# googlegenomics/spark-examples

Measured on NVIDIA H100. Metric: genotype-cells/sec (N x V) into Gram, higher is better.
Workload: dtype int8

## Files before the change

spark_examples_b200/csrc/gram_sm90.cu:

```cuda
#include <cuda.h>
#include <cuda_runtime.h>

#include <cstring>

#include <algorithm>
#include <map>
#include <mutex>
#include <tuple>
#include <type_traits>
#include <cstdio>
#include <cstdlib>
#include <string>
#include <vector>

#include "ptx_sm90.cuh"
#include "vpca_internal.h"

namespace vpca {

namespace {

constexpr int kThreads = 384;
constexpr int kKBytes = 128;
constexpr int kBoxRows = 128;
// ... 451 lines not shown
                const int rowA = (CG == 2 && cta_rank != 0) ? s.rowA1 : s.rowA0;
                const bool two_boxes = s.n_eff > kBoxRows;
                const bool self_b = (CG == 2) && (s.flags & kTileSelfB) != 0;
                const uint32_t tx = (uint32_t)((two_boxes ? 2 : 1) + (self_b ? 0 : 1)) * C::BOX_BYTES;
                if (a.sync_lead > 0 && leader && s.win != synced_win) {
                    synced_win = s.win;
                    if (s.win >= a.sync_lead) wait_window(a.win_done, s.win - a.sync_lead, a.active_workers);
                }
                for (int kb = s.kb0; kb < s.kb1; ++kb, ++it) {
                    const uint32_t st = it % C::STAGES, ph = (it / C::STAGES) & 1u;
                    mbar_wait(empty_bar(st), ph ^ 1u, a.err, 1);
                    const int pnl = kb / a.kb_per_panel;
                    const int kc = (kb - pnl * a.kb_per_panel) * a.kc_per_kb;
                    ptx::mbar_arrive_expect_tx(full_bar(st), tx);
                    if constexpr (CG == 2) {
                        if (two_boxes || cta_rank == 0)
                            ptx::tma_load_3d_multicast(sB(st) + cta_rank * C::BOX_BYTES, &tmap, full_bar(st), kc,
                                                       s.rowB + (int)cta_rank * kBoxRows, pnl, 0x3);
                    } else {
                        ptx::tma_load_3d(sB(st), &tmap, full_bar(st), kc, s.rowB, pnl);
                        if (two_boxes) ptx::tma_load_3d(sB(st) + C::BOX_BYTES, &tmap, full_bar(st), kc, s.rowB + kBoxRows, pnl);
                    }
                    if (!self_b) ptx::tma_load_3d(sA(st), &tmap, full_bar(st), kc, rowA, pnl);
                }
                if (a.sync_lead > 0 && leader && s.last_in_win)
                    asm volatile("red.release.gpu.global.add.s32 [%0], 1;" ::"l"(a.win_done + s.win) : "memory");
            }
        }
    } else {
        asm volatile("setmaxnreg.inc.sync.aligned.u32 232;");
        const int cw = (warp >> 2) - 1;
        const int wq = warp & 3;
        const uint32_t ctid = threadIdx.x - 128;
        AccT<KIND> acc[2][64];
        Sched sc;
        sc.init(a, worker);
        Seg s;
        uint32_t it = 0;
        while (sc.next(s)) {
            const bool filler = (CG == 2) && cta_rank != 0 && (s.flags & kTileFiller) != 0;
            const bool self_b = (CG == 2) && (s.flags & kTileSelfB) != 0;
            const int mrow0 = cw * 128;
            const bool act0 = mrow0 < s.n_eff, act1 = mrow0 + 64 < s.n_eff;
            if (s.first) {
#pragma unroll
                for (int i = 0; i < 64; ++i) {
                    acc[0][i] = 0;
                    acc[1][i] = 0;
                }
            }
            const uint32_t a_off = (self_b ? cta_rank : 2u) * (uint32_t)(kBoxRows * 128);
            int pending = -1;
            for (int kb = s.kb0; kb < s.kb1; ++kb, ++it) {
                const uint32_t st = it % C::STAGES, ph = (it / C::STAGES) & 1u;
                mbar_wait(full_bar(st), ph, a.err, 3);
                uint32_t opB, opA;
                if constexpr (KIND == 2) {
                    const uint32_t xb = smem_base + C::STAGES * C::STAGE_BYTES + (it & 1u) * C::XBUF_BYTES;
                    ptx::named_sync(1, 256);
                    const int nb = s.n_eff > kBoxRows ? 2 * kBoxRows : kBoxRows;
                    const int rows = nb + (self_b ? 0 : kBoxRows);
                    for (int c = (int)ctid; c < rows * 8; c += 256) {
                        const int r = c >> 3, j = c & 7;
                        const uint32_t src = (r < nb ? sB(st) + (uint32_t)r * 64u : sA(st) + (uint32_t)(r - nb) * 64u) + (uint32_t)j * 8u;
                        const int xr = r < nb ? r : 2 * kBoxRows + (r - nb);
                        uint32_t lo, hi;
                        asm volatile("ld.shared.v2.u32 {%0, %1}, [%2];" : "=r"(lo), "=r"(hi) : "r"(src));
                        const uint32_t o0 = e2m1x4_to_s8x2(lo & 0xFFFFu), o1 = e2m1x4_to_s8x2(lo >> 16);
                        const uint32_t o2 = e2m1x4_to_s8x2(hi & 0xFFFFu), o3 = e2m1x4_to_s8x2(hi >> 16);
                        const uint32_t dst = xb + (uint32_t)xr * 128u + (((uint32_t)j ^ ((uint32_t)xr & 7u)) << 4);
                        asm volatile("st.shared.v4.u32 [%0], {%1, %2, %3, %4};" ::"r"(dst), "r"(o0), "r"(o1), "r"(o2), "r"(o3)
                                     : "memory");
                    }
                    ptx::fence_proxy_async();
                    ptx::named_sync(1, 256);
                    if (threadIdx.x % 128 == 0) release(st);
                    opB = xb;
                } else {
                    opB = sB(st);
                }
                opA = opB + a_off;
                const uint64_t bdesc = make_smem_desc(opA);
                const uint64_t adesc0 = make_smem_desc(opB + (uint32_t)mrow0 * 128u);
                const uint64_t adesc1 = make_smem_desc(opB + (uint32_t)(mrow0 + 64) * 128u);
                ptx::wgmma_fence_acc(acc[0]);
                ptx::wgmma_fence_acc(acc[1]);
                ptx::wgmma_fence();
#pragma unroll
                for (int k = 0; k < kKBytes / 32; ++k) {
                    if constexpr (KIND == 1) {
                        ptx::wgmma_bf16(acc[0], adesc0 + 2 * k, bdesc + 2 * k);
                        ptx::wgmma_bf16(acc[1], adesc1 + 2 * k, bdesc + 2 * k);
                    } else {
                        ptx::wgmma_s8(acc[0], adesc0 + 2 * k, bdesc + 2 * k);
                        ptx::wgmma_s8(acc[1], adesc1 + 2 * k, bdesc + 2 * k);
                    }
                }
                ptx::wgmma_commit();
                ptx::wgmma_wait<1>();
                ptx::wgmma_fence_acc(acc[0]);
                ptx::wgmma_fence_acc(acc[1]);
                if constexpr (KIND != 2) {
                    if (pending >= 0 && threadIdx.x % 128 == 0) release((uint32_t)pending);
                }
                pending = (int)st;
            }
            ptx::wgmma_wait<0>();
            ptx::wgmma_fence_acc(acc[0]);
            ptx::wgmma_fence_acc(acc[1]);
            if constexpr (KIND != 2) {
                if (pending >= 0 && threadIdx.x % 128 == 0) release((uint32_t)pending);
            }
            if (!s.flush || filler) continue;

            const int colA = (CG == 2 && cta_rank != 0) ? s.rowA1 : s.rowA0;
            const int row_end = min(a.row_limit, s.rowB + s.n_eff);
            const bool pair64 = a.red64 != 0 && (a.n & 1) == 0;
#pragma unroll
            for (int j = 0; j < 2; ++j) {
                if (!(j == 0 ? act0 : act1)) continue;
#pragma unroll
                for (int h = 0; h < 2; ++h) {
                    const int row = s.rowB + mrow0 + 64 * j + 16 * wq + (int)(lane >> 2) + 8 * h;
                    if (row >= row_end) continue;
                    int32_t* own = a.S;
                    if (a.num_peers != 0 && a.peer_mode == 1) {
                        int o = 0;
                        while (o + 1 < a.num_peers && row >= a.own_end[o]) ++o;
                        own = a.peer[o];
                    }
#pragma unroll
                    for (int i = 0; i < 16; ++i) {
                        const int col = colA + 8 * i + 2 * (int)(lane & 3);
                        if (col >= a.n) continue;
                        int v0 = acc_to_int<KIND>(acc[j][4 * i + 2 * h]);
                        int v1 = acc_to_int<KIND>(acc[j][4 * i + 2 * h + 1]);
                        if ((s.flags & kTileXpose) != 0 && (row >> 7) < (col >> 7)) {
                            for (int e = 0; e < 2; ++e) {
                                const int v = e ? v1 : v0, c = col + e;
                                if (v == 0 || c >= a.n) continue;
                                const size_t o = (size_t)c * (size_t)a.n + (size_t)row;
                                if (a.num_peers == 0) {
                                    asm volatile("red.global.add.s32 [%0], %1;" ::"l"(a.S + o), "r"(v) : "memory");
                                } else if (a.peer_mode == 1) {
                                    int q = 0;
                                    while (q + 1 < a.num_peers && c >= a.own_end[q]) ++q;
                                    asm volatile("red.relaxed.sys.global.add.s32 [%0], %1;" ::"l"(a.peer[q] + o), "r"(v) : "memory");
                                } else {
                                    for (int d = 0; d < a.num_peers; ++d)
                                        asm volatile("red.relaxed.sys.global.add.s32 [%0], %1;" ::"l"(a.peer[d] + o), "r"(v)
                                                     : "memory");
                                }
                            }
                            continue;
                        }
                        if (row < col) v0 = 0;
                        if (row < col + 1 || col + 1 >= a.n) v1 = 0;
                        if ((v0 | v1) == 0) continue;
                        const size_t o = (size_t)row * (size_t)a.n + (size_t)col;
                        if (pair64) {
                            const unsigned long long packed = (unsigned long long)(unsigned)v0 | ((unsigned long long)(unsigned)v1 << 32);
                            if (a.num_peers == 0) {
                                asm volatile("red.global.add.u64 [%0], %1;" ::"l"(a.S + o), "l"(packed) : "memory");
                            } else if (a.peer_mode == 1) {
                                asm volatile("red.relaxed.sys.global.add.u64 [%0], %1;" ::"l"(own + o), "l"(packed) : "memory");
                            } else {
                                for (int d = 0; d < a.num_peers; ++d)
                                    asm volatile("red.relaxed.sys.global.add.u64 [%0], %1;" ::"l"(a.peer[d] + o), "l"(packed)
                                                 : "memory");
                            }
                        } else {
                            for (int e = 0; e < 2; ++e) {
                                const int v = e ? v1 : v0;
                                if (v == 0) continue;
                                if (a.num_peers == 0) {
                                    asm volatile("red.global.add.s32 [%0], %1;" ::"l"(a.S + o + e), "r"(v) : "memory");
                                } else if (a.peer_mode == 1) {
                                    asm volatile("red.relaxed.sys.global.add.s32 [%0], %1;" ::"l"(own + o + e), "r"(v) : "memory");
                                } else {
                                    for (int d = 0; d < a.num_peers; ++d)
                                        asm volatile("red.relaxed.sys.global.add.s32 [%0], %1;" ::"l"(a.peer[d] + o + e), "r"(v)
                                                     : "memory");
                                }
                            }
                        }
                    }
                }
            }
        }
        if (a.prof != nullptr && threadIdx.x == 128) a.prof[(size_t)blockIdx.x * 4 + 2] = globaltimer_ns();
    }

    if constexpr (CG == 2) ptx::cluster_sync();
    else __syncthreads();
    if (a.prof != nullptr && threadIdx.x == 0) a.prof[(size_t)blockIdx.x * 4 + 3] = globaltimer_ns();
}

__global__ void rebalance_kernel(const long long* __restrict__ prof, double* __restrict__ cum, int workers, int cta_group,
                                 double gain, double max_share, long long min_ns, int* __restrict__ gen, const TileDesc* __restrict__ tiles,
                                 int num_tiles, int total_weight, int kbw, int col_limit) {
    __shared__ double sh[1024];
    __shared__ double cand[1025];
    __shared__ long long need[1025];
    __shared__ double red_sum, red_min;
    __shared__ int reject, need_repair;
    const int w = threadIdx.x;
    const bool active = w < workers;
    double t = 0.0, share_old = 0.0;
    if (active) {
        const long long t0 = prof[(size_t)w * cta_group * 4 + 0], t1 = prof[(size_t)w * cta_group * 4 + 2];
        t = (double)(t1 - t0);
        share_old = cum[w + 1] - cum[w];
    }
    sh[w] = active ? t : 1e30;
    if (w == 0) {
        reject = 0;
// ... 865 lines not shown
```

spark_examples_b200/csrc/ptx_sm90.cuh:

```cuda
#pragma once
#include <cstdint>
#include <cuda_runtime.h>

namespace vpca {
namespace ptx {

__device__ __forceinline__ uint32_t smem_u32(const void* p) {
    return static_cast<uint32_t>(__cvta_generic_to_shared(p));
}

__device__ __forceinline__ uint32_t lane_id() {
    uint32_t r;
    asm volatile("mov.u32 %0, %%laneid;" : "=r"(r));
    return r;
}

__device__ __forceinline__ bool elect_one() {
    uint32_t pred = 0;
    asm volatile(
        "{\n\t"
        ".reg .pred P;\n\t"
        "elect.sync _|P, 0xffffffff;\n\t"
        "selp.u32 %0, 1, 0, P;\n\t"
        "}\n"
// ... 33 lines not shown
__device__ __forceinline__ void prefetch_tensormap(const void* desc) {
    asm volatile("prefetch.tensormap [%0];" ::"l"(reinterpret_cast<uint64_t>(desc)) : "memory");
}
__device__ __forceinline__ void tma_load_3d(uint32_t smem_dst, const void* desc, uint32_t bar, int32_t c0, int32_t c1,
                                            int32_t c2) {
    asm volatile(
        "cp.async.bulk.tensor.3d.shared::cluster.global.mbarrier::complete_tx::bytes [%0], [%1, {%3, %4, %5}], [%2];"
        ::"r"(smem_dst), "l"(reinterpret_cast<uint64_t>(desc)), "r"(bar), "r"(c0), "r"(c1), "r"(c2)
        : "memory");
}
__device__ __forceinline__ void tma_load_3d_multicast(uint32_t smem_dst, const void* desc, uint32_t bar, int32_t c0,
                                                      int32_t c1, int32_t c2, uint16_t cta_mask) {
    asm volatile(
        "cp.async.bulk.tensor.3d.shared::cluster.global.mbarrier::complete_tx::bytes.multicast::cluster"
        " [%0], [%1, {%3, %4, %5}], [%2], %6;"
        ::"r"(smem_dst), "l"(reinterpret_cast<uint64_t>(desc)), "r"(bar), "r"(c0), "r"(c1), "r"(c2), "h"(cta_mask)
        : "memory");
}
__device__ __forceinline__ uint32_t mapa(uint32_t saddr, uint32_t rank) {
    uint32_t r;
    asm volatile("mapa.shared::cluster.u32 %0, %1, %2;" : "=r"(r) : "r"(saddr), "r"(rank));
    return r;
}
__device__ __forceinline__ void mbar_arrive_cluster(uint32_t cluster_bar) {
    asm volatile("mbarrier.arrive.shared::cluster.b64 _, [%0];" ::"r"(cluster_bar) : "memory");
}
__device__ __forceinline__ void cluster_sync() {
    asm volatile("barrier.cluster.arrive.release;\n\tbarrier.cluster.wait.acquire;" ::: "memory");
}
__device__ __forceinline__ void wgmma_fence() { asm volatile("wgmma.fence.sync.aligned;" ::: "memory"); }
__device__ __forceinline__ void wgmma_commit() { asm volatile("wgmma.commit_group.sync.aligned;" ::: "memory"); }
template <int N>
__device__ __forceinline__ void wgmma_wait() { asm volatile("wgmma.wait_group.sync.aligned %0;" ::"n"(N) : "memory"); }
__device__ __forceinline__ void wgmma_fence_acc(uint32_t (&d)[64]) {
#pragma unroll
    for (int i = 0; i < 64; ++i) asm volatile("" : "+r"(d[i])::"memory");
}
__device__ __forceinline__ void wgmma_fence_acc(float (&d)[64]) {
#pragma unroll
    for (int i = 0; i < 64; ++i) asm volatile("" : "+f"(d[i])::"memory");
}

__device__ __forceinline__ void wgmma_s8(uint32_t (&d)[64], uint64_t a_desc, uint64_t b_desc) {
    asm volatile(
        "{\n\t.reg .pred p;\n\tsetp.ne.b32 p, 1, 0;\n\t"
        "wgmma.mma_async.sync.aligned.m64n128k32.s32.s8.s8 "
        "{%0, %1, %2, %3, %4, %5, %6, %7, %8, %9, %10, %11, %12, %13, %14, %15, %16, %17, %18, %19, %20, %21, %22, %23, %24, %25, %26, %27, %28, %29, %30, %31, %32, %33, %34, %35, %36, %37, %38, %39, %40, %41, %42, %43, %44, %45, %46, %47, %48, %49, %50, %51, %52, %53, %54, %55, %56, %57, %58, %59, %60, %61, %62, %63}, %64, %65, p;\n\t}\n"
        : "+r"(d[0]), "+r"(d[1]), "+r"(d[2]), "+r"(d[3]), "+r"(d[4]), "+r"(d[5]), "+r"(d[6]), "+r"(d[7]), "+r"(d[8]), "+r"(d[9]), "+r"(d[10]), "+r"(d[11]), "+r"(d[12]), "+r"(d[13]), "+r"(d[14]), "+r"(d[15]), "+r"(d[16]), "+r"(d[17]), "+r"(d[18]), "+r"(d[19]), "+r"(d[20]), "+r"(d[21]), "+r"(d[22]), "+r"(d[23]), "+r"(d[24]), "+r"(d[25]), "+r"(d[26]), "+r"(d[27]), "+r"(d[28]), "+r"(d[29]), "+r"(d[30]), "+r"(d[31]), "+r"(d[32]), "+r"(d[33]), "+r"(d[34]), "+r"(d[35]), "+r"(d[36]), "+r"(d[37]), "+r"(d[38]), "+r"(d[39]), "+r"(d[40]), "+r"(d[41]), "+r"(d[42]), "+r"(d[43]), "+r"(d[44]), "+r"(d[45]), "+r"(d[46]), "+r"(d[47]), "+r"(d[48]), "+r"(d[49]), "+r"(d[50]), "+r"(d[51]), "+r"(d[52]), "+r"(d[53]), "+r"(d[54]), "+r"(d[55]), "+r"(d[56]), "+r"(d[57]), "+r"(d[58]), "+r"(d[59]), "+r"(d[60]), "+r"(d[61]), "+r"(d[62]), "+r"(d[63])
        : "l"(a_desc), "l"(b_desc));
}

__device__ __forceinline__ void wgmma_bf16(float (&f)[64], uint64_t a_desc, uint64_t b_desc) {
    asm volatile(
        "{\n\t.reg .pred p;\n\tsetp.ne.b32 p, 1, 0;\n\t"
        "wgmma.mma_async.sync.aligned.m64n128k16.f32.bf16.bf16 "
        "{%0, %1, %2, %3, %4, %5, %6, %7, %8, %9, %10, %11, %12, %13, %14, %15, %16, %17, %18, %19, %20, %21, %22, %23, %24, %25, %26, %27, %28, %29, %30, %31, %32, %33, %34, %35, %36, %37, %38, %39, %40, %41, %42, %43, %44, %45, %46, %47, %48, %49, %50, %51, %52, %53, %54, %55, %56, %57, %58, %59, %60, %61, %62, %63}, %64, %65, p, 1, 1, 0, 0;\n\t}\n"
        : "+f"(f[0]), "+f"(f[1]), "+f"(f[2]), "+f"(f[3]), "+f"(f[4]), "+f"(f[5]), "+f"(f[6]), "+f"(f[7]), "+f"(f[8]), "+f"(f[9]), "+f"(f[10]), "+f"(f[11]), "+f"(f[12]), "+f"(f[13]), "+f"(f[14]), "+f"(f[15]), "+f"(f[16]), "+f"(f[17]), "+f"(f[18]), "+f"(f[19]), "+f"(f[20]), "+f"(f[21]), "+f"(f[22]), "+f"(f[23]), "+f"(f[24]), "+f"(f[25]), "+f"(f[26]), "+f"(f[27]), "+f"(f[28]), "+f"(f[29]), "+f"(f[30]), "+f"(f[31]), "+f"(f[32]), "+f"(f[33]), "+f"(f[34]), "+f"(f[35]), "+f"(f[36]), "+f"(f[37]), "+f"(f[38]), "+f"(f[39]), "+f"(f[40]), "+f"(f[41]), "+f"(f[42]), "+f"(f[43]), "+f"(f[44]), "+f"(f[45]), "+f"(f[46]), "+f"(f[47]), "+f"(f[48]), "+f"(f[49]), "+f"(f[50]), "+f"(f[51]), "+f"(f[52]), "+f"(f[53]), "+f"(f[54]), "+f"(f[55]), "+f"(f[56]), "+f"(f[57]), "+f"(f[58]), "+f"(f[59]), "+f"(f[60]), "+f"(f[61]), "+f"(f[62]), "+f"(f[63])
        : "l"(a_desc), "l"(b_desc));
}

__device__ __forceinline__ void named_sync(uint32_t id, uint32_t count) {
    asm volatile("bar.sync %0, %1;" ::"r"(id), "r"(count) : "memory");
}

}
}
```

Before: 627.6 billion.

## Swap wgmma operand roles to use m64n256 instructions per consumer warpgroup

Each consumer warpgroup now issues one m64n256 wgmma per k-step, with the A-side (64 rows per warpgroup) as the M operand and the full 256-row B block as N. Before, it issued two m64n128 wgmmas sharing a B descriptor. Because the accumulator is now transposed, the epilogue uses a lane-pair shuffle to rebuild adjacent column pairs so the atomic reductions stay paired. The intent is to halve wgmma issue count and make better use of shared-memory operand bandwidth. In exchange the epilogue gets extra shuffles and per-row bounds checks, and tiles with fewer than 256 active rows still compute all 256 columns.

```diff
diff --git a/spark_examples_b200/csrc/gram_sm90.cu b/spark_examples_b200/csrc/gram_sm90.cu
--- a/spark_examples_b200/csrc/gram_sm90.cu
+++ b/spark_examples_b200/csrc/gram_sm90.cu
@@ -507,29 +507,19 @@
         const int cw = (warp >> 2) - 1;
         const int wq = warp & 3;
         const uint32_t ctid = threadIdx.x - 128;
-        AccT<KIND> acc[2][64];
+        AccT<KIND> acc[128];
         Sched sc;
         sc.init(a, worker);
-        Seg s;
+        Seg s{};
         uint32_t it = 0;
-        while (sc.next(s)) {
-            const bool filler = (CG == 2) && cta_rank != 0 && (s.flags & kTileFiller) != 0;
-            const bool self_b = (CG == 2) && (s.flags & kTileSelfB) != 0;
-            const int mrow0 = cw * 128;
-            const bool act0 = mrow0 < s.n_eff, act1 = mrow0 + 64 < s.n_eff;
-            if (s.first) {
-#pragma unroll
-                for (int i = 0; i < 64; ++i) {
-                    acc[0][i] = 0;
-                    acc[1][i] = 0;
-                }
-            }
-            const uint32_t a_off = (self_b ? cta_rank : 2u) * (uint32_t)(kBoxRows * 128);
+        auto consume = [&](auto n_const, uint32_t it, uint32_t a_off, uint32_t b_off, bool self_b) {
+            constexpr int N = decltype(n_const)::value;
             int pending = -1;
-            for (int kb = s.kb0; kb < s.kb1; ++kb, ++it) {
+            const uint32_t it_end = it + (uint32_t)(s.kb1 - s.kb0);
+            for (; it != it_end; ++it) {
                 const uint32_t st = it % C::STAGES, ph = (it / C::STAGES) & 1u;
                 mbar_wait(full_bar(st), ph, a.err, 3);
-                uint32_t opB, opA;
+                uint32_t opB;
                 if constexpr (KIND == 2) {
                     const uint32_t xb = smem_base + C::STAGES * C::STAGE_BYTES + (it & 1u) * C::XBUF_BYTES;
                     ptx::named_sync(1, 256);
@@ -554,109 +544,112 @@
                 } else {
                     opB = sB(st);
                 }
-                opA = opB + a_off;
-                const uint64_t bdesc = make_smem_desc(opA);
-                const uint64_t adesc0 = make_smem_desc(opB + (uint32_t)mrow0 * 128u);
-                const uint64_t adesc1 = make_smem_desc(opB + (uint32_t)(mrow0 + 64) * 128u);
-                ptx::wgmma_fence_acc(acc[0]);
-                ptx::wgmma_fence_acc(acc[1]);
-                ptx::wgmma_fence();
+                if constexpr (N > 0) {
+                    const uint64_t adesc = make_smem_desc(opB + a_off);
+                    const uint64_t bdesc = make_smem_desc(opB + b_off);
+                    ptx::wgmma_fence_acc<N>(acc);
+                    ptx::wgmma_fence();
 #pragma unroll
-                for (int k = 0; k < kKBytes / 32; ++k) {
-                    if constexpr (KIND == 1) {
-                        ptx::wgmma_bf16(acc[0], adesc0 + 2 * k, bdesc + 2 * k);
-                        ptx::wgmma_bf16(acc[1], adesc1 + 2 * k, bdesc + 2 * k);
-                    } else {
-                        ptx::wgmma_s8(acc[0], adesc0 + 2 * k, bdesc + 2 * k);
-                        ptx::wgmma_s8(acc[1], adesc1 + 2 * k, bdesc + 2 * k);
+                    for (int k = 0; k < kKBytes / 32; ++k) {
+                        if constexpr (KIND == 1) ptx::wgmma_bf16<N>(acc, adesc + 2 * k, bdesc + 2 * k);
+                        else ptx::wgmma_s8<N>(acc, adesc + 2 * k, bdesc + 2 * k);
                     }
+                    ptx::wgmma_commit();
+                    ptx::wgmma_wait<1>();
+                    ptx::wgmma_fence_acc<N>(acc);
                 }
-                ptx::wgmma_commit();
-                ptx::wgmma_wait<1>();
-                ptx::wgmma_fence_acc(acc[0]);
-                ptx::wgmma_fence_acc(acc[1]);
                 if constexpr (KIND != 2) {
                     if (pending >= 0 && threadIdx.x % 128 == 0) release((uint32_t)pending);
                 }
                 pending = (int)st;
             }
-            ptx::wgmma_wait<0>();
-            ptx::wgmma_fence_acc(acc[0]);
-            ptx::wgmma_fence_acc(acc[1]);
+            if constexpr (N > 0) {
+                ptx::wgmma_wait<0>();
+                ptx::wgmma_fence_acc<N>(acc);
+            }
             if constexpr (KIND != 2) {
                 if (pending >= 0 && threadIdx.x % 128 == 0) release((uint32_t)pending);
             }
+            return it;
+        };
+        while (sc.next(s)) {
+            const bool filler = (CG == 2) && cta_rank != 0 && (s.flags & kTileFiller) != 0;
+            const bool self_b = (CG == 2) && (s.flags & kTileSelfB) != 0;
+            if (s.first) {
+#pragma unroll
+                for (int i = 0; i < 128; ++i) acc[i] = 0;
+            }
+            const uint32_t a_off = ((self_b ? cta_rank : 2u) * (uint32_t)kBoxRows + (uint32_t)(64 * cw)) * 128u;
+            it = consume(std::integral_constant<int, 256>{}, it, a_off, 0u, self_b);
             if (!s.flush || filler) continue;
 
-            const int colA = (CG == 2 && cta_rank != 0) ? s.rowA1 : s.rowA0;
+            const int colA = ((CG == 2 && cta_rank != 0) ? s.rowA1 : s.rowA0) + 64 * cw;
             const int row_end = min(a.row_limit, s.rowB + s.n_eff);
             const bool pair64 = a.red64 != 0 && (a.n & 1) == 0;
+            const uint32_t odd = (lane >> 2) & 1u;
 #pragma unroll
-            for (int j = 0; j < 2; ++j) {
-                if (!(j == 0 ? act0 : act1)) continue;
+            for (int i = 0; i < 32; ++i) {
+                if (s.rowB + 8 * i >= row_end) break;
 #pragma unroll
                 for (int h = 0; h < 2; ++h) {
-                    const int row = s.rowB + mrow0 + 64 * j + 16 * wq + (int)(lane >> 2) + 8 * h;
-                    if (row >= row_end) continue;
+                    const int m0 = acc_to_int<KIND>(acc[4 * i + 2 * h]), m1 = acc_to_int<KIND>(acc[4 * i + 2 * h + 1]);
+                    const int got = __shfl_xor_sync(0xffffffffu, odd ? m0 : m1, 4);
+                    int v0 = odd ? got : m0, v1 = odd ? m1 : got;
+                    const int row = s.rowB + 8 * i + 2 * (int)(lane & 3) + (int)odd;
+                    const int col = colA + 16 * wq + (int)((lane >> 2) & ~1u) + 8 * h;
+                    if (row >= row_end || col >= a.n) continue;
                     int32_t* own = a.S;
                     if (a.num_peers != 0 && a.peer_mode == 1) {
                         int o = 0;
                         while (o + 1 < a.num_peers && row >= a.own_end[o]) ++o;
                         own = a.peer[o];
                     }
-#pragma unroll
-                    for (int i = 0; i < 16; ++i) {
-                        const int col = colA + 8 * i + 2 * (int)(lane & 3);
-                        if (col >= a.n) continue;
-                        int v0 = acc_to_int<KIND>(acc[j][4 * i + 2 * h]);
-                        int v1 = acc_to_int<KIND>(acc[j][4 * i + 2 * h + 1]);
-                        if ((s.flags & kTileXpose) != 0 && (row >> 7) < (col >> 7)) {
-                            for (int e = 0; e < 2; ++e) {
-                                const int v = e ? v1 : v0, c = col + e;
-                                if (v == 0 || c >= a.n) continue;
-                                const size_t o = (size_t)c * (size_t)a.n + (size_t)row;
-                                if (a.num_peers == 0) {
-                                    asm volatile("red.global.add.s32 [%0], %1;" ::"l"(a.S + o), "r"(v) : "memory");
-                                } else if (a.peer_mode == 1) {
-                                    int q = 0;
-                                    while (q + 1 < a.num_peers && c >= a.own_end[q]) ++q;
-                                    asm volatile("red.relaxed.sys.global.add.s32 [%0], %1;" ::"l"(a.peer[q] + o), "r"(v) : "memory");
-                                } else {
-                                    for (int d = 0; d < a.num_peers; ++d)
-                                        asm volatile("red.relaxed.sys.global.add.s32 [%0], %1;" ::"l"(a.peer[d] + o), "r"(v)
-                                                     : "memory");
-                                }
-                            }
-                            continue;
-                        }
-                        if (row < col) v0 = 0;
-                        if (row < col + 1 || col + 1 >= a.n) v1 = 0;
-                        if ((v0 | v1) == 0) continue;
-                        const size_t o = (size_t)row * (size_t)a.n + (size_t)col;
-                        if (pair64) {
-                            const unsigned long long packed = (unsigned long long)(unsigned)v0 | ((unsigned long long)(unsigned)v1 << 32);
+                    if ((s.flags & kTileXpose) != 0 && (row >> 7) < (col >> 7)) {
+                        for (int e = 0; e < 2; ++e) {
+                            const int v = e ? v1 : v0, c = col + e;
+                            if (v == 0 || c >= a.n) continue;
+                            const size_t o = (size_t)c * (size_t)a.n + (size_t)row;
                             if (a.num_peers == 0) {
-                                asm volatile("red.global.add.u64 [%0], %1;" ::"l"(a.S + o), "l"(packed) : "memory");
+                                asm volatile("red.global.add.s32 [%0], %1;" ::"l"(a.S + o), "r"(v) : "memory");
                             } else if (a.peer_mode == 1) {
-                                asm volatile("red.relaxed.sys.global.add.u64 [%0], %1;" ::"l"(own + o), "l"(packed) : "memory");
+                                int q = 0;
+                                while (q + 1 < a.num_peers && c >= a.own_end[q]) ++q;
+                                asm volatile("red.relaxed.sys.global.add.s32 [%0], %1;" ::"l"(a.peer[q] + o), "r"(v) : "memory");
                             } else {
                                 for (int d = 0; d < a.num_peers; ++d)
-                                    asm volatile("red.relaxed.sys.global.add.u64 [%0], %1;" ::"l"(a.peer[d] + o), "l"(packed)
+                                    asm volatile("red.relaxed.sys.global.add.s32 [%0], %1;" ::"l"(a.peer[d] + o), "r"(v)
                                                  : "memory");
                             }
+                        }
+                        continue;
+                    }
+                    if (row < col) v0 = 0;
+                    if (row < col + 1 || col + 1 >= a.n) v1 = 0;
+                    if ((v0 | v1) == 0) continue;
+                    const size_t o = (size_t)row * (size_t)a.n + (size_t)col;
+                    if (pair64) {
+                        const unsigned long long packed = (unsigned long long)(unsigned)v0 | ((unsigned long long)(unsigned)v1 << 32);
+                        if (a.num_peers == 0) {
+                            asm volatile("red.global.add.u64 [%0], %1;" ::"l"(a.S + o), "l"(packed) : "memory");
+                        } else if (a.peer_mode == 1) {
+                            asm volatile("red.relaxed.sys.global.add.u64 [%0], %1;" ::"l"(own + o), "l"(packed) : "memory");
                         } else {
-                            for (int e = 0; e < 2; ++e) {
-                                const int v = e ? v1 : v0;
-                                if (v == 0) continue;
-                                if (a.num_peers == 0) {
-                                    asm volatile("red.global.add.s32 [%0], %1;" ::"l"(a.S + o + e), "r"(v) : "memory");
-                                } else if (a.peer_mode == 1) {
-                                    asm volatile("red.relaxed.sys.global.add.s32 [%0], %1;" ::"l"(own + o + e), "r"(v) : "memory");
-                                } else {
-                                    for (int d = 0; d < a.num_peers; ++d)
-                                        asm volatile("red.relaxed.sys.global.add.s32 [%0], %1;" ::"l"(a.peer[d] + o + e), "r"(v)
-                                                     : "memory");
-                                }
+                            for (int d = 0; d < a.num_peers; ++d)
+                                asm volatile("red.relaxed.sys.global.add.u64 [%0], %1;" ::"l"(a.peer[d] + o), "l"(packed)
+                                             : "memory");
+                        }
+                    } else {
+                        for (int e = 0; e < 2; ++e) {
+                            const int v = e ? v1 : v0;
+                            if (v == 0) continue;
+                            if (a.num_peers == 0) {
+                                asm volatile("red.global.add.s32 [%0], %1;" ::"l"(a.S + o + e), "r"(v) : "memory");
+                            } else if (a.peer_mode == 1) {
+                                asm volatile("red.relaxed.sys.global.add.s32 [%0], %1;" ::"l"(own + o + e), "r"(v) : "memory");
+                            } else {
+                                for (int d = 0; d < a.num_peers; ++d)
+                                    asm volatile("red.relaxed.sys.global.add.s32 [%0], %1;" ::"l"(a.peer[d] + o + e), "r"(v)
+                                                 : "memory");
                             }
                         }
                     }
diff --git a/spark_examples_b200/csrc/ptx_sm90.cuh b/spark_examples_b200/csrc/ptx_sm90.cuh
--- a/spark_examples_b200/csrc/ptx_sm90.cuh
+++ b/spark_examples_b200/csrc/ptx_sm90.cuh
@@ -89,32 +89,72 @@
 __device__ __forceinline__ void wgmma_commit() { asm volatile("wgmma.commit_group.sync.aligned;" ::: "memory"); }
 template <int N>
 __device__ __forceinline__ void wgmma_wait() { asm volatile("wgmma.wait_group.sync.aligned %0;" ::"n"(N) : "memory"); }
-__device__ __forceinline__ void wgmma_fence_acc(uint32_t (&d)[64]) {
+template <int N>
+__device__ __forceinline__ void wgmma_fence_acc(uint32_t (&d)[128]) {
 #pragma unroll
-    for (int i = 0; i < 64; ++i) asm volatile("" : "+r"(d[i])::"memory");
+    for (int i = 0; i < N / 2; ++i) asm volatile("" : "+r"(d[i])::"memory");
 }
-__device__ __forceinline__ void wgmma_fence_acc(float (&d)[64]) {
+template <int N>
+__device__ __forceinline__ void wgmma_fence_acc(float (&d)[128]) {
 #pragma unroll
-    for (int i = 0; i < 64; ++i) asm volatile("" : "+f"(d[i])::"memory");
+    for (int i = 0; i < N / 2; ++i) asm volatile("" : "+f"(d[i])::"memory");
 }
 
-__device__ __forceinline__ void wgmma_s8(uint32_t (&d)[64], uint64_t a_desc, uint64_t b_desc) {
-    asm volatile(
-        "{\n\t.reg .pred p;\n\tsetp.ne.b32 p, 1, 0;\n\t"
-        "wgmma.mma_async.sync.aligned.m64n128k32.s32.s8.s8 "
-        "{%0, %1, %2, %3, %4, %5, %6, %7, %8, %9, %10, %11, %12, %13, %14, %15, %16, %17, %18, %19, %20, %21, %22, %23, %24, %25, %26, %27, %28, %29, %30, %31, %32, %33, %34, %35, %36, %37, %38, %39, %40, %41, %42, %43, %44, %45, %46, %47, %48, %49, %50, %51, %52, %53, %54, %55, %56, %57, %58, %59, %60, %61, %62, %63}, %64, %65, p;\n\t}\n"
-        : "+r"(d[0]), "+r"(d[1]), "+r"(d[2]), "+r"(d[3]), "+r"(d[4]), "+r"(d[5]), "+r"(d[6]), "+r"(d[7]), "+r"(d[8]), "+r"(d[9]), "+r"(d[10]), "+r"(d[11]), "+r"(d[12]), "+r"(d[13]), "+r"(d[14]), "+r"(d[15]), "+r"(d[16]), "+r"(d[17]), "+r"(d[18]), "+r"(d[19]), "+r"(d[20]), "+r"(d[21]), "+r"(d[22]), "+r"(d[23]), "+r"(d[24]), "+r"(d[25]), "+r"(d[26]), "+r"(d[27]), "+r"(d[28]), "+r"(d[29]), "+r"(d[30]), "+r"(d[31]), "+r"(d[32]), "+r"(d[33]), "+r"(d[34]), "+r"(d[35]), "+r"(d[36]), "+r"(d[37]), "+r"(d[38]), "+r"(d[39]), "+r"(d[40]), "+r"(d[41]), "+r"(d[42]), "+r"(d[43]), "+r"(d[44]), "+r"(d[45]), "+r"(d[46]), "+r"(d[47]), "+r"(d[48]), "+r"(d[49]), "+r"(d[50]), "+r"(d[51]), "+r"(d[52]), "+r"(d[53]), "+r"(d[54]), "+r"(d[55]), "+r"(d[56]), "+r"(d[57]), "+r"(d[58]), "+r"(d[59]), "+r"(d[60]), "+r"(d[61]), "+r"(d[62]), "+r"(d[63])
-        : "l"(a_desc), "l"(b_desc));
+#define VPCA_WG_D16 "%0, %1, %2, %3, %4, %5, %6, %7"
+#define VPCA_WG_D32 VPCA_WG_D16 ", %8, %9, %10, %11, %12, %13, %14, %15"
+#define VPCA_WG_D48 VPCA_WG_D32 ", %16, %17, %18, %19, %20, %21, %22, %23"
+#define VPCA_WG_D64 VPCA_WG_D48 ", %24, %25, %26, %27, %28, %29, %30, %31"
+#define VPCA_WG_D80 VPCA_WG_D64 ", %32, %33, %34, %35, %36, %37, %38, %39"
+#define VPCA_WG_D96 VPCA_WG_D80 ", %40, %41, %42, %43, %44, %45, %46, %47"
+#define VPCA_WG_D112 VPCA_WG_D96 ", %48, %49, %50, %51, %52, %53, %54, %55"
+#define VPCA_WG_D128 VPCA_WG_D112 ", %56, %57, %58, %59, %60, %61, %62, %63"
+#define VPCA_WG_D144 VPCA_WG_D128 ", %64, %65, %66, %67, %68, %69, %70, %71"
+#define VPCA_WG_D160 VPCA_WG_D144 ", %72, %73, %74, %75, %76, %77, %78, %79"
+#define VPCA_WG_D176 VPCA_WG_D160 ", %80, %81, %82, %83, %84, %85, %86, %87"
+#define VPCA_WG_D192 VPCA_WG_D176 ", %88, %89, %90, %91, %92, %93, %94, %95"
+#define VPCA_WG_D208 VPCA_WG_D192 ", %96, %97, %98, %99, %100, %101, %102, %103"
+#define VPCA_WG_D224 VPCA_WG_D208 ", %104, %105, %106, %107, %108, %109, %110, %111"
+#define VPCA_WG_D240 VPCA_WG_D224 ", %112, %113, %114, %115, %116, %117, %118, %119"
+#define VPCA_WG_D256 VPCA_WG_D240 ", %120, %121, %122, %123, %124, %125, %126, %127"
+#define VPCA_WG_OP8(C, d, i) C(d[i]), C(d[i + 1]), C(d[i + 2]), C(d[i + 3]), C(d[i + 4]), C(d[i + 5]), C(d[i + 6]), C(d[i + 7])
+#define VPCA_WG_OPS(C, d)                                                                                                  \
+    VPCA_WG_OP8(C, d, 0), VPCA_WG_OP8(C, d, 8), VPCA_WG_OP8(C, d, 16), VPCA_WG_OP8(C, d, 24), VPCA_WG_OP8(C, d, 32),      \
+        VPCA_WG_OP8(C, d, 40), VPCA_WG_OP8(C, d, 48), VPCA_WG_OP8(C, d, 56), VPCA_WG_OP8(C, d, 64), VPCA_WG_OP8(C, d, 72), \
+        VPCA_WG_OP8(C, d, 80), VPCA_WG_OP8(C, d, 88), VPCA_WG_OP8(C, d, 96), VPCA_WG_OP8(C, d, 104),                      \
+        VPCA_WG_OP8(C, d, 112), VPCA_WG_OP8(C, d, 120)
+#define VPCA_WG_S8(NN)                                                                                         \
+    if constexpr (N == NN)                                                                                     \
+        asm volatile("{\n\t.reg .pred p;\n\tsetp.ne.b32 p, 1, 0;\n\t"                                          \
+                     "wgmma.mma_async.sync.aligned.m64n" #NN "k32.s32.s8.s8 {" VPCA_WG_D##NN "}, %128, %129, p;\n\t}\n" \
+                     : VPCA_WG_OPS("+r", d)                                                                    \
+                     : "l"(a_desc), "l"(b_desc));
+#define VPCA_WG_BF16(NN)                                                                                       \
+    if constexpr (N == NN)                                                                                     \
+        asm volatile("{\n\t.reg .pred p;\n\tsetp.ne.b32 p, 1, 0;\n\t"                                          \
+                     "wgmma.mma_async.sync.aligned.m64n" #NN "k16.f32.bf16.bf16 {" VPCA_WG_D##NN                \
+                     "}, %128, %129, p, 1, 1, 0, 0;\n\t}\n"                                                    \
+                     : VPCA_WG_OPS("+f", f)                                                                    \
+                     : "l"(a_desc), "l"(b_desc));
+
+template <int N>
+__device__ __forceinline__ void wgmma_s8(uint32_t (&d)[128], uint64_t a_desc, uint64_t b_desc) {
+    static_assert(N % 16 == 0 && N >= 16 && N <= 256, "wgmma_s8: N is a multiple of 16 in [16, 256]");
+    VPCA_WG_S8(16) VPCA_WG_S8(32) VPCA_WG_S8(48) VPCA_WG_S8(64) VPCA_WG_S8(80) VPCA_WG_S8(96) VPCA_WG_S8(112)
+    VPCA_WG_S8(128) VPCA_WG_S8(144) VPCA_WG_S8(160) VPCA_WG_S8(176) VPCA_WG_S8(192) VPCA_WG_S8(208) VPCA_WG_S8(224)
+    VPCA_WG_S8(240) VPCA_WG_S8(256)
 }
 
-__device__ __forceinline__ void wgmma_bf16(float (&f)[64], uint64_t a_desc, uint64_t b_desc) {
-    asm volatile(
-        "{\n\t.reg .pred p;\n\tsetp.ne.b32 p, 1, 0;\n\t"
-        "wgmma.mma_async.sync.aligned.m64n128k16.f32.bf16.bf16 "
-        "{%0, %1, %2, %3, %4, %5, %6, %7, %8, %9, %10, %11, %12, %13, %14, %15, %16, %17, %18, %19, %20, %21, %22, %23, %24, %25, %26, %27, %28, %29, %30, %31, %32, %33, %34, %35, %36, %37, %38, %39, %40, %41, %42, %43, %44, %45, %46, %47, %48, %49, %50, %51, %52, %53, %54, %55, %56, %57, %58, %59, %60, %61, %62, %63}, %64, %65, p, 1, 1, 0, 0;\n\t}\n"
-        : "+f"(f[0]), "+f"(f[1]), "+f"(f[2]), "+f"(f[3]), "+f"(f[4]), "+f"(f[5]), "+f"(f[6]), "+f"(f[7]), "+f"(f[8]), "+f"(f[9]), "+f"(f[10]), "+f"(f[11]), "+f"(f[12]), "+f"(f[13]), "+f"(f[14]), "+f"(f[15]), "+f"(f[16]), "+f"(f[17]), "+f"(f[18]), "+f"(f[19]), "+f"(f[20]), "+f"(f[21]), "+f"(f[22]), "+f"(f[23]), "+f"(f[24]), "+f"(f[25]), "+f"(f[26]), "+f"(f[27]), "+f"(f[28]), "+f"(f[29]), "+f"(f[30]), "+f"(f[31]), "+f"(f[32]), "+f"(f[33]), "+f"(f[34]), "+f"(f[35]), "+f"(f[36]), "+f"(f[37]), "+f"(f[38]), "+f"(f[39]), "+f"(f[40]), "+f"(f[41]), "+f"(f[42]), "+f"(f[43]), "+f"(f[44]), "+f"(f[45]), "+f"(f[46]), "+f"(f[47]), "+f"(f[48]), "+f"(f[49]), "+f"(f[50]), "+f"(f[51]), "+f"(f[52]), "+f"(f[53]), "+f"(f[54]), "+f"(f[55]), "+f"(f[56]), "+f"(f[57]), "+f"(f[58]), "+f"(f[59]), "+f"(f[60]), "+f"(f[61]), "+f"(f[62]), "+f"(f[63])
-        : "l"(a_desc), "l"(b_desc));
+template <int N>
+__device__ __forceinline__ void wgmma_bf16(float (&f)[128], uint64_t a_desc, uint64_t b_desc) {
+    static_assert(N % 16 == 0 && N >= 16 && N <= 256, "wgmma_bf16: N is a multiple of 16 in [16, 256]");
+    VPCA_WG_BF16(16) VPCA_WG_BF16(32) VPCA_WG_BF16(48) VPCA_WG_BF16(64) VPCA_WG_BF16(80) VPCA_WG_BF16(96)
+    VPCA_WG_BF16(112) VPCA_WG_BF16(128) VPCA_WG_BF16(144) VPCA_WG_BF16(160) VPCA_WG_BF16(176) VPCA_WG_BF16(192)
+    VPCA_WG_BF16(208) VPCA_WG_BF16(224) VPCA_WG_BF16(240) VPCA_WG_BF16(256)
 }
+#undef VPCA_WG_S8
+#undef VPCA_WG_BF16
+#undef VPCA_WG_OPS
+#undef VPCA_WG_OP8
 
 __device__ __forceinline__ void named_sync(uint32_t id, uint32_t count) {
     asm volatile("bar.sync %0, %1;" ::"r"(id), "r"(count) : "memory");
```

After: 642.8 billion (median of 6 runs). 2.4% higher.

## Switch consumer WGMMA to m64n256 with swapped operand roles and transposed epilogue

Applied to the files above, without the earlier changes.

Each consumer warpgroup now issues one m64n256k32 WGMMA per k-step instead of two m64n128 instructions. The roles flip: the 128-row A tile supplies 64 rows per warpgroup and the full 256-row B panel becomes the N dimension. This halves the WGMMA instruction count and cuts redundant shared-memory reads of the shared operand. The accumulator is now transposed relative to the output, so the epilogue uses a lane-xor-4 shuffle to rebuild adjacent column pairs for the packed 64-bit reductions. The cost is more complex epilogue indexing, and per-row masking based on n_eff no longer skips whole inactive 64-row halves.

```diff
diff --git a/spark_examples_b200/csrc/gram_sm90.cu b/spark_examples_b200/csrc/gram_sm90.cu
--- a/spark_examples_b200/csrc/gram_sm90.cu
+++ b/spark_examples_b200/csrc/gram_sm90.cu
@@ -507,7 +507,7 @@
         const int cw = (warp >> 2) - 1;
         const int wq = warp & 3;
         const uint32_t ctid = threadIdx.x - 128;
-        AccT<KIND> acc[2][64];
+        AccT<KIND> acc[128];
         Sched sc;
         sc.init(a, worker);
         Seg s;
@@ -515,14 +515,9 @@
         while (sc.next(s)) {
             const bool filler = (CG == 2) && cta_rank != 0 && (s.flags & kTileFiller) != 0;
             const bool self_b = (CG == 2) && (s.flags & kTileSelfB) != 0;
-            const int mrow0 = cw * 128;
-            const bool act0 = mrow0 < s.n_eff, act1 = mrow0 + 64 < s.n_eff;
             if (s.first) {
 #pragma unroll
-                for (int i = 0; i < 64; ++i) {
-                    acc[0][i] = 0;
-                    acc[1][i] = 0;
-                }
+                for (int i = 0; i < 128; ++i) acc[i] = 0;
             }
             const uint32_t a_off = (self_b ? cta_rank : 2u) * (uint32_t)(kBoxRows * 128);
             int pending = -1;
@@ -555,34 +550,25 @@
                     opB = sB(st);
                 }
                 opA = opB + a_off;
-                const uint64_t bdesc = make_smem_desc(opA);
-                const uint64_t adesc0 = make_smem_desc(opB + (uint32_t)mrow0 * 128u);
-                const uint64_t adesc1 = make_smem_desc(opB + (uint32_t)(mrow0 + 64) * 128u);
-                ptx::wgmma_fence_acc(acc[0]);
-                ptx::wgmma_fence_acc(acc[1]);
+                const uint64_t adesc = make_smem_desc(opA + (uint32_t)cw * 64u * 128u);
+                const uint64_t bdesc = make_smem_desc(opB);
+                ptx::wgmma_fence_acc(acc);
                 ptx::wgmma_fence();
 #pragma unroll
                 for (int k = 0; k < kKBytes / 32; ++k) {
-                    if constexpr (KIND == 1) {
-                        ptx::wgmma_bf16(acc[0], adesc0 + 2 * k, bdesc + 2 * k);
-                        ptx::wgmma_bf16(acc[1], adesc1 + 2 * k, bdesc + 2 * k);
-                    } else {
-                        ptx::wgmma_s8(acc[0], adesc0 + 2 * k, bdesc + 2 * k);
-                        ptx::wgmma_s8(acc[1], adesc1 + 2 * k, bdesc + 2 * k);
-                    }
+                    if constexpr (KIND == 1) ptx::wgmma_bf16(acc, adesc + 2 * k, bdesc + 2 * k);
+                    else ptx::wgmma_s8(acc, adesc + 2 * k, bdesc + 2 * k);
                 }
                 ptx::wgmma_commit();
                 ptx::wgmma_wait<1>();
-                ptx::wgmma_fence_acc(acc[0]);
-                ptx::wgmma_fence_acc(acc[1]);
+                ptx::wgmma_fence_acc(acc);
                 if constexpr (KIND != 2) {
                     if (pending >= 0 && threadIdx.x % 128 == 0) release((uint32_t)pending);
                 }
                 pending = (int)st;
             }
             ptx::wgmma_wait<0>();
-            ptx::wgmma_fence_acc(acc[0]);
-            ptx::wgmma_fence_acc(acc[1]);
+            ptx::wgmma_fence_acc(acc);
             if constexpr (KIND != 2) {
                 if (pending >= 0 && threadIdx.x % 128 == 0) release((uint32_t)pending);
             }
@@ -591,72 +577,71 @@
             const int colA = (CG == 2 && cta_rank != 0) ? s.rowA1 : s.rowA0;
             const int row_end = min(a.row_limit, s.rowB + s.n_eff);
             const bool pair64 = a.red64 != 0 && (a.n & 1) == 0;
+            const bool upper = (lane & 4u) != 0;
 #pragma unroll
-            for (int j = 0; j < 2; ++j) {
-                if (!(j == 0 ? act0 : act1)) continue;
+            for (int h = 0; h < 2; ++h) {
+                const int col = colA + 64 * cw + 16 * wq + (int)((lane >> 2) & ~1u) + 8 * h;
 #pragma unroll
-                for (int h = 0; h < 2; ++h) {
-                    const int row = s.rowB + mrow0 + 64 * j + 16 * wq + (int)(lane >> 2) + 8 * h;
-                    if (row >= row_end) continue;
+                for (int i = 0; i < 64; ++i) {
+                    const int c0 = acc_to_int<KIND>(acc[4 * i + 2 * h]);
+                    const int c1 = acc_to_int<KIND>(acc[4 * i + 2 * h + 1]);
+                    const int peer = __shfl_xor_sync(0xffffffffu, upper ? c0 : c1, 4);
+                    int v0 = upper ? peer : c0;
+                    int v1 = upper ? c1 : peer;
+                    const int row = s.rowB + 8 * i + 2 * (int)(lane & 3) + (upper ? 1 : 0);
+                    if (row >= row_end || col >= a.n) continue;
+                    if ((s.flags & kTileXpose) != 0 && (row >> 7) < (col >> 7)) {
+                        for (int e = 0; e < 2; ++e) {
+                            const int v = e ? v1 : v0, c = col + e;
+                            if (v == 0 || c >= a.n) continue;
+                            const size_t o = (size_t)(unsigned)c * (unsigned)a.n + (unsigned)row;
+                            if (a.num_peers == 0) {
+                                asm volatile("red.global.add.s32 [%0], %1;" ::"l"(a.S + o), "r"(v) : "memory");
+                            } else if (a.peer_mode == 1) {
+                                int q = 0;
+                                while (q + 1 < a.num_peers && c >= a.own_end[q]) ++q;
+                                asm volatile("red.relaxed.sys.global.add.s32 [%0], %1;" ::"l"(a.peer[q] + o), "r"(v) : "memory");
+                            } else {
+                                for (int d = 0; d < a.num_peers; ++d)
+                                    asm volatile("red.relaxed.sys.global.add.s32 [%0], %1;" ::"l"(a.peer[d] + o), "r"(v)
+                                                 : "memory");
+                            }
+                        }
+                        continue;
+                    }
+                    if (row < col) v0 = 0;
+                    if (row < col + 1 || col + 1 >= a.n) v1 = 0;
+                    if ((v0 | v1) == 0) continue;
                     int32_t* own = a.S;
                     if (a.num_peers != 0 && a.peer_mode == 1) {
                         int o = 0;
                         while (o + 1 < a.num_peers && row >= a.own_end[o]) ++o;
                         own = a.peer[o];
                     }
-#pragma unroll
-                    for (int i = 0; i < 16; ++i) {
-                        const int col = colA + 8 * i + 2 * (int)(lane & 3);
-                        if (col >= a.n) continue;
-                        int v0 = acc_to_int<KIND>(acc[j][4 * i + 2 * h]);
-                        int v1 = acc_to_int<KIND>(acc[j][4 * i + 2 * h + 1]);
-                        if ((s.flags & kTileXpose) != 0 && (row >> 7) < (col >> 7)) {
-                            for (int e = 0; e < 2; ++e) {
-                                const int v = e ? v1 : v0, c = col + e;
-                                if (v == 0 || c >= a.n) continue;
-                                const size_t o = (size_t)c * (size_t)a.n + (size_t)row;
-                                if (a.num_peers == 0) {
-                                    asm volatile("red.global.add.s32 [%0], %1;" ::"l"(a.S + o), "r"(v) : "memory");
-                                } else if (a.peer_mode == 1) {
-                                    int q = 0;
-                                    while (q + 1 < a.num_peers && c >= a.own_end[q]) ++q;
-                                    asm volatile("red.relaxed.sys.global.add.s32 [%0], %1;" ::"l"(a.peer[q] + o), "r"(v) : "memory");
-                                } else {
-                                    for (int d = 0; d < a.num_peers; ++d)
-                                        asm volatile("red.relaxed.sys.global.add.s32 [%0], %1;" ::"l"(a.peer[d] + o), "r"(v)
-                                                     : "memory");
-                                }
-                            }
-                            continue;
+                    const size_t o = (size_t)(unsigned)row * (unsigned)a.n + (unsigned)col;
+                    if (pair64) {
+                        const unsigned long long packed = (unsigned long long)(unsigned)v0 | ((unsigned long long)(unsigned)v1 << 32);
+                        if (a.num_peers == 0) {
+                            asm volatile("red.global.add.u64 [%0], %1;" ::"l"(a.S + o), "l"(packed) : "memory");
+                        } else if (a.peer_mode == 1) {
+                            asm volatile("red.relaxed.sys.global.add.u64 [%0], %1;" ::"l"(own + o), "l"(packed) : "memory");
+                        } else {
+                            for (int d = 0; d < a.num_peers; ++d)
+                                asm volatile("red.relaxed.sys.global.add.u64 [%0], %1;" ::"l"(a.peer[d] + o), "l"(packed)
+                                             : "memory");
                         }
-                        if (row < col) v0 = 0;
-                        if (row < col + 1 || col + 1 >= a.n) v1 = 0;
-                        if ((v0 | v1) == 0) continue;
-                        const size_t o = (size_t)row * (size_t)a.n + (size_t)col;
-                        if (pair64) {
-                            const unsigned long long packed = (unsigned long long)(unsigned)v0 | ((unsigned long long)(unsigned)v1 << 32);
+                    } else {
+                        for (int e = 0; e < 2; ++e) {
+                            const int v = e ? v1 : v0;
+                            if (v == 0) continue;
                             if (a.num_peers == 0) {
-                                asm volatile("red.global.add.u64 [%0], %1;" ::"l"(a.S + o), "l"(packed) : "memory");
+                                asm volatile("red.global.add.s32 [%0], %1;" ::"l"(a.S + o + e), "r"(v) : "memory");
                             } else if (a.peer_mode == 1) {
-                                asm volatile("red.relaxed.sys.global.add.u64 [%0], %1;" ::"l"(own + o), "l"(packed) : "memory");
+                                asm volatile("red.relaxed.sys.global.add.s32 [%0], %1;" ::"l"(own + o + e), "r"(v) : "memory");
                             } else {
                                 for (int d = 0; d < a.num_peers; ++d)
-                                    asm volatile("red.relaxed.sys.global.add.u64 [%0], %1;" ::"l"(a.peer[d] + o), "l"(packed)
+                                    asm volatile("red.relaxed.sys.global.add.s32 [%0], %1;" ::"l"(a.peer[d] + o + e), "r"(v)
                                                  : "memory");
-                            }
-                        } else {
-                            for (int e = 0; e < 2; ++e) {
-                                const int v = e ? v1 : v0;
-                                if (v == 0) continue;
-                                if (a.num_peers == 0) {
-                                    asm volatile("red.global.add.s32 [%0], %1;" ::"l"(a.S + o + e), "r"(v) : "memory");
-                                } else if (a.peer_mode == 1) {
-                                    asm volatile("red.relaxed.sys.global.add.s32 [%0], %1;" ::"l"(own + o + e), "r"(v) : "memory");
-                                } else {
-                                    for (int d = 0; d < a.num_peers; ++d)
-                                        asm volatile("red.relaxed.sys.global.add.s32 [%0], %1;" ::"l"(a.peer[d] + o + e), "r"(v)
-                                                     : "memory");
-                                }
                             }
                         }
                     }
diff --git a/spark_examples_b200/csrc/ptx_sm90.cuh b/spark_examples_b200/csrc/ptx_sm90.cuh
--- a/spark_examples_b200/csrc/ptx_sm90.cuh
+++ b/spark_examples_b200/csrc/ptx_sm90.cuh
@@ -89,30 +89,30 @@
 __device__ __forceinline__ void wgmma_commit() { asm volatile("wgmma.commit_group.sync.aligned;" ::: "memory"); }
 template <int N>
 __device__ __forceinline__ void wgmma_wait() { asm volatile("wgmma.wait_group.sync.aligned %0;" ::"n"(N) : "memory"); }
-__device__ __forceinline__ void wgmma_fence_acc(uint32_t (&d)[64]) {
+__device__ __forceinline__ void wgmma_fence_acc(uint32_t (&d)[128]) {
 #pragma unroll
-    for (int i = 0; i < 64; ++i) asm volatile("" : "+r"(d[i])::"memory");
+    for (int i = 0; i < 128; ++i) asm volatile("" : "+r"(d[i])::"memory");
 }
-__device__ __forceinline__ void wgmma_fence_acc(float (&d)[64]) {
+__device__ __forceinline__ void wgmma_fence_acc(float (&d)[128]) {
 #pragma unroll
-    for (int i = 0; i < 64; ++i) asm volatile("" : "+f"(d[i])::"memory");
+    for (int i = 0; i < 128; ++i) asm volatile("" : "+f"(d[i])::"memory");
 }
 
-__device__ __forceinline__ void wgmma_s8(uint32_t (&d)[64], uint64_t a_desc, uint64_t b_desc) {
+__device__ __forceinline__ void wgmma_s8(uint32_t (&d)[128], uint64_t a_desc, uint64_t b_desc) {
     asm volatile(
         "{\n\t.reg .pred p;\n\tsetp.ne.b32 p, 1, 0;\n\t"
-        "wgmma.mma_async.sync.aligned.m64n128k32.s32.s8.s8 "
-        "{%0, %1, %2, %3, %4, %5, %6, %7, %8, %9, %10, %11, %12, %13, %14, %15, %16, %17, %18, %19, %20, %21, %22, %23, %24, %25, %26, %27, %28, %29, %30, %31, %32, %33, %34, %35, %36, %37, %38, %39, %40, %41, %42, %43, %44, %45, %46, %47, %48, %49, %50, %51, %52, %53, %54, %55, %56, %57, %58, %59, %60, %61, %62, %63}, %64, %65, p;\n\t}\n"
-        : "+r"(d[0]), "+r"(d[1]), "+r"(d[2]), "+r"(d[3]), "+r"(d[4]), "+r"(d[5]), "+r"(d[6]), "+r"(d[7]), "+r"(d[8]), "+r"(d[9]), "+r"(d[10]), "+r"(d[11]), "+r"(d[12]), "+r"(d[13]), "+r"(d[14]), "+r"(d[15]), "+r"(d[16]), "+r"(d[17]), "+r"(d[18]), "+r"(d[19]), "+r"(d[20]), "+r"(d[21]), "+r"(d[22]), "+r"(d[23]), "+r"(d[24]), "+r"(d[25]), "+r"(d[26]), "+r"(d[27]), "+r"(d[28]), "+r"(d[29]), "+r"(d[30]), "+r"(d[31]), "+r"(d[32]), "+r"(d[33]), "+r"(d[34]), "+r"(d[35]), "+r"(d[36]), "+r"(d[37]), "+r"(d[38]), "+r"(d[39]), "+r"(d[40]), "+r"(d[41]), "+r"(d[42]), "+r"(d[43]), "+r"(d[44]), "+r"(d[45]), "+r"(d[46]), "+r"(d[47]), "+r"(d[48]), "+r"(d[49]), "+r"(d[50]), "+r"(d[51]), "+r"(d[52]), "+r"(d[53]), "+r"(d[54]), "+r"(d[55]), "+r"(d[56]), "+r"(d[57]), "+r"(d[58]), "+r"(d[59]), "+r"(d[60]), "+r"(d[61]), "+r"(d[62]), "+r"(d[63])
+        "wgmma.mma_async.sync.aligned.m64n256k32.s32.s8.s8 "
+        "{%0, %1, %2, %3, %4, %5, %6, %7, %8, %9, %10, %11, %12, %13, %14, %15, %16, %17, %18, %19, %20, %21, %22, %23, %24, %25, %26, %27, %28, %29, %30, %31, %32, %33, %34, %35, %36, %37, %38, %39, %40, %41, %42, %43, %44, %45, %46, %47, %48, %49, %50, %51, %52, %53, %54, %55, %56, %57, %58, %59, %60, %61, %62, %63, %64, %65, %66, %67, %68, %69, %70, %71, %72, %73, %74, %75, %76, %77, %78, %79, %80, %81, %82, %83, %84, %85, %86, %87, %88, %89, %90, %91, %92, %93, %94, %95, %96, %97, %98, %99, %100, %101, %102, %103, %104, %105, %106, %107, %108, %109, %110, %111, %112, %113, %114, %115, %116, %117, %118, %119, %120, %121, %122, %123, %124, %125, %126, %127}, %128, %129, p;\n\t}\n"
+        : "+r"(d[0]), "+r"(d[1]), "+r"(d[2]), "+r"(d[3]), "+r"(d[4]), "+r"(d[5]), "+r"(d[6]), "+r"(d[7]), "+r"(d[8]), "+r"(d[9]), "+r"(d[10]), "+r"(d[11]), "+r"(d[12]), "+r"(d[13]), "+r"(d[14]), "+r"(d[15]), "+r"(d[16]), "+r"(d[17]), "+r"(d[18]), "+r"(d[19]), "+r"(d[20]), "+r"(d[21]), "+r"(d[22]), "+r"(d[23]), "+r"(d[24]), "+r"(d[25]), "+r"(d[26]), "+r"(d[27]), "+r"(d[28]), "+r"(d[29]), "+r"(d[30]), "+r"(d[31]), "+r"(d[32]), "+r"(d[33]), "+r"(d[34]), "+r"(d[35]), "+r"(d[36]), "+r"(d[37]), "+r"(d[38]), "+r"(d[39]), "+r"(d[40]), "+r"(d[41]), "+r"(d[42]), "+r"(d[43]), "+r"(d[44]), "+r"(d[45]), "+r"(d[46]), "+r"(d[47]), "+r"(d[48]), "+r"(d[49]), "+r"(d[50]), "+r"(d[51]), "+r"(d[52]), "+r"(d[53]), "+r"(d[54]), "+r"(d[55]), "+r"(d[56]), "+r"(d[57]), "+r"(d[58]), "+r"(d[59]), "+r"(d[60]), "+r"(d[61]), "+r"(d[62]), "+r"(d[63]), "+r"(d[64]), "+r"(d[65]), "+r"(d[66]), "+r"(d[67]), "+r"(d[68]), "+r"(d[69]), "+r"(d[70]), "+r"(d[71]), "+r"(d[72]), "+r"(d[73]), "+r"(d[74]), "+r"(d[75]), "+r"(d[76]), "+r"(d[77]), "+r"(d[78]), "+r"(d[79]), "+r"(d[80]), "+r"(d[81]), "+r"(d[82]), "+r"(d[83]), "+r"(d[84]), "+r"(d[85]), "+r"(d[86]), "+r"(d[87]), "+r"(d[88]), "+r"(d[89]), "+r"(d[90]), "+r"(d[91]), "+r"(d[92]), "+r"(d[93]), "+r"(d[94]), "+r"(d[95]), "+r"(d[96]), "+r"(d[97]), "+r"(d[98]), "+r"(d[99]), "+r"(d[100]), "+r"(d[101]), "+r"(d[102]), "+r"(d[103]), "+r"(d[104]), "+r"(d[105]), "+r"(d[106]), "+r"(d[107]), "+r"(d[108]), "+r"(d[109]), "+r"(d[110]), "+r"(d[111]), "+r"(d[112]), "+r"(d[113]), "+r"(d[114]), "+r"(d[115]), "+r"(d[116]), "+r"(d[117]), "+r"(d[118]), "+r"(d[119]), "+r"(d[120]), "+r"(d[121]), "+r"(d[122]), "+r"(d[123]), "+r"(d[124]), "+r"(d[125]), "+r"(d[126]), "+r"(d[127])
         : "l"(a_desc), "l"(b_desc));
 }
 
-__device__ __forceinline__ void wgmma_bf16(float (&f)[64], uint64_t a_desc, uint64_t b_desc) {
+__device__ __forceinline__ void wgmma_bf16(float (&f)[128], uint64_t a_desc, uint64_t b_desc) {
     asm volatile(
         "{\n\t.reg .pred p;\n\tsetp.ne.b32 p, 1, 0;\n\t"
-        "wgmma.mma_async.sync.aligned.m64n128k16.f32.bf16.bf16 "
-        "{%0, %1, %2, %3, %4, %5, %6, %7, %8, %9, %10, %11, %12, %13, %14, %15, %16, %17, %18, %19, %20, %21, %22, %23, %24, %25, %26, %27, %28, %29, %30, %31, %32, %33, %34, %35, %36, %37, %38, %39, %40, %41, %42, %43, %44, %45, %46, %47, %48, %49, %50, %51, %52, %53, %54, %55, %56, %57, %58, %59, %60, %61, %62, %63}, %64, %65, p, 1, 1, 0, 0;\n\t}\n"
-        : "+f"(f[0]), "+f"(f[1]), "+f"(f[2]), "+f"(f[3]), "+f"(f[4]), "+f"(f[5]), "+f"(f[6]), "+f"(f[7]), "+f"(f[8]), "+f"(f[9]), "+f"(f[10]), "+f"(f[11]), "+f"(f[12]), "+f"(f[13]), "+f"(f[14]), "+f"(f[15]), "+f"(f[16]), "+f"(f[17]), "+f"(f[18]), "+f"(f[19]), "+f"(f[20]), "+f"(f[21]), "+f"(f[22]), "+f"(f[23]), "+f"(f[24]), "+f"(f[25]), "+f"(f[26]), "+f"(f[27]), "+f"(f[28]), "+f"(f[29]), "+f"(f[30]), "+f"(f[31]), "+f"(f[32]), "+f"(f[33]), "+f"(f[34]), "+f"(f[35]), "+f"(f[36]), "+f"(f[37]), "+f"(f[38]), "+f"(f[39]), "+f"(f[40]), "+f"(f[41]), "+f"(f[42]), "+f"(f[43]), "+f"(f[44]), "+f"(f[45]), "+f"(f[46]), "+f"(f[47]), "+f"(f[48]), "+f"(f[49]), "+f"(f[50]), "+f"(f[51]), "+f"(f[52]), "+f"(f[53]), "+f"(f[54]), "+f"(f[55]), "+f"(f[56]), "+f"(f[57]), "+f"(f[58]), "+f"(f[59]), "+f"(f[60]), "+f"(f[61]), "+f"(f[62]), "+f"(f[63])
+        "wgmma.mma_async.sync.aligned.m64n256k16.f32.bf16.bf16 "
+        "{%0, %1, %2, %3, %4, %5, %6, %7, %8, %9, %10, %11, %12, %13, %14, %15, %16, %17, %18, %19, %20, %21, %22, %23, %24, %25, %26, %27, %28, %29, %30, %31, %32, %33, %34, %35, %36, %37, %38, %39, %40, %41, %42, %43, %44, %45, %46, %47, %48, %49, %50, %51, %52, %53, %54, %55, %56, %57, %58, %59, %60, %61, %62, %63, %64, %65, %66, %67, %68, %69, %70, %71, %72, %73, %74, %75, %76, %77, %78, %79, %80, %81, %82, %83, %84, %85, %86, %87, %88, %89, %90, %91, %92, %93, %94, %95, %96, %97, %98, %99, %100, %101, %102, %103, %104, %105, %106, %107, %108, %109, %110, %111, %112, %113, %114, %115, %116, %117, %118, %119, %120, %121, %122, %123, %124, %125, %126, %127}, %128, %129, p, 1, 1, 0, 0;\n\t}\n"
+        : "+f"(f[0]), "+f"(f[1]), "+f"(f[2]), "+f"(f[3]), "+f"(f[4]), "+f"(f[5]), "+f"(f[6]), "+f"(f[7]), "+f"(f[8]), "+f"(f[9]), "+f"(f[10]), "+f"(f[11]), "+f"(f[12]), "+f"(f[13]), "+f"(f[14]), "+f"(f[15]), "+f"(f[16]), "+f"(f[17]), "+f"(f[18]), "+f"(f[19]), "+f"(f[20]), "+f"(f[21]), "+f"(f[22]), "+f"(f[23]), "+f"(f[24]), "+f"(f[25]), "+f"(f[26]), "+f"(f[27]), "+f"(f[28]), "+f"(f[29]), "+f"(f[30]), "+f"(f[31]), "+f"(f[32]), "+f"(f[33]), "+f"(f[34]), "+f"(f[35]), "+f"(f[36]), "+f"(f[37]), "+f"(f[38]), "+f"(f[39]), "+f"(f[40]), "+f"(f[41]), "+f"(f[42]), "+f"(f[43]), "+f"(f[44]), "+f"(f[45]), "+f"(f[46]), "+f"(f[47]), "+f"(f[48]), "+f"(f[49]), "+f"(f[50]), "+f"(f[51]), "+f"(f[52]), "+f"(f[53]), "+f"(f[54]), "+f"(f[55]), "+f"(f[56]), "+f"(f[57]), "+f"(f[58]), "+f"(f[59]), "+f"(f[60]), "+f"(f[61]), "+f"(f[62]), "+f"(f[63]), "+f"(f[64]), "+f"(f[65]), "+f"(f[66]), "+f"(f[67]), "+f"(f[68]), "+f"(f[69]), "+f"(f[70]), "+f"(f[71]), "+f"(f[72]), "+f"(f[73]), "+f"(f[74]), "+f"(f[75]), "+f"(f[76]), "+f"(f[77]), "+f"(f[78]), "+f"(f[79]), "+f"(f[80]), "+f"(f[81]), "+f"(f[82]), "+f"(f[83]), "+f"(f[84]), "+f"(f[85]), "+f"(f[86]), "+f"(f[87]), "+f"(f[88]), "+f"(f[89]), "+f"(f[90]), "+f"(f[91]), "+f"(f[92]), "+f"(f[93]), "+f"(f[94]), "+f"(f[95]), "+f"(f[96]), "+f"(f[97]), "+f"(f[98]), "+f"(f[99]), "+f"(f[100]), "+f"(f[101]), "+f"(f[102]), "+f"(f[103]), "+f"(f[104]), "+f"(f[105]), "+f"(f[106]), "+f"(f[107]), "+f"(f[108]), "+f"(f[109]), "+f"(f[110]), "+f"(f[111]), "+f"(f[112]), "+f"(f[113]), "+f"(f[114]), "+f"(f[115]), "+f"(f[116]), "+f"(f[117]), "+f"(f[118]), "+f"(f[119]), "+f"(f[120]), "+f"(f[121]), "+f"(f[122]), "+f"(f[123]), "+f"(f[124]), "+f"(f[125]), "+f"(f[126]), "+f"(f[127])
         : "l"(a_desc), "l"(b_desc));
 }
 
```

Result: faster. 626.4 billion before, 634.0 billion after, median of 6 (+1.2%).
